# yzhang511/multi_modal_foundation_model

Hardware: AMD Instinct MI355X
Metric: pretrain samples/sec (T=100 bins/modality, d_model=256, 5+5 layers, spike+behaviour masked pretraining step) (higher is better)
Workload: dtype bf16; 1 GPU; BASELINE.json configs[1]: 1 session, ap(668 neurons)+behaviour(2), d_model=256, heads=8, mlp=512, 5 enc + 5 dec layers, T=100 (L=200 tokens), dropout 0.4/0.2, AdamW+OneCycleLR, mixed objectives; per_gpu_batch=1024, global_batch=1024, seq_len=200, parallelism=dp1

## Files before the change

### include/mmfm.h

```cpp
#ifndef MMFM_H
#define MMFM_H
#include <stdint.h>
#ifdef __cplusplus
extern "C" {
#endif

#define MMFM_VERSION 401
#define MMFM_F32 0
#define MMFM_BF16 1
#define MMFM_NULL_BIAS 1
#define MMFM_EMBED_OPTS 1
#define MMFM_MLP_GELU 0
#define MMFM_MLP_RELU 1
#define MMFM_MLP_SIGMOID 2
#define MMFM_MLP_GELU_TANH 3

typedef void* mmfm_stream;

typedef struct {
    const void* state;
    uint32_t site;
    float p;
} mmfm_dropout;

// ... 179 lines not shown
    int K, N;
    const void* x; int ldx;
    const void* w; int ldw;
    const float* bias;
    int ln; float eps;
    void* xhat; float* rstd;
    const void* residual; int ldr;
    void* y; int ldy;
    int stream_out;
    int rotate;
    int ln_bwd;
    const void* bwd_xhat; const float* bwd_rstd;
} mmfm_rowgemm_desc;
int mmfm_rowgemm(const mmfm_rowgemm_desc* d, mmfm_stream stream);

typedef struct {
    int64_t R;
    const void* x; int ldx;
    float eps;
    const void* w_up; const float* b_up;
    const void* w_down; const float* b_down;
    mmfm_dropout drop;
    void* y; int ldy;
    void* xhat; float* rstd;
    const void* dy; int lddy;
    const void* w_down_t;
    const void* w_up_t;
    void* t1; void* g; void* du;
    void* dx; int lddx;
    int rotate;
// ... 22 lines not shown
```

### multi_modal_foundation_model_amd/_lib.py

```python
from __future__ import annotations

import ctypes as C
import os
import re

import torch

_HERE = os.path.dirname(os.path.abspath(__file__))
LIB_PATH = os.environ.get("MMFM_LIB") or os.path.join(_HERE, "libmmfm_hip.so")
HEADER_PATH = os.path.join(os.path.dirname(_HERE), "include", "mmfm.h")

F32, BF16 = 0, 1
ATTN_DIAG, ATTN_CAUSAL, ATTN_SEP = 1, 2, 4
ACT_NONE, ACT_GELU, ACT_SOFTSIGN, ACT_GELU_GRAD, ACT_SOFTSIGN_GRAD, ACT_SOFTSIGN_GRAD_OUT = 0, 1, 2, 3, 4, 5
ACT_RELU, ACT_RELU_GRAD, ACT_SIGMOID, ACT_SIGMOID_GRAD, ACT_GELU_TANH, ACT_GELU_TANH_GRAD = 6, 7, 8, 9, 10, 11
(ACT_EMB_IDENTITY, ACT_EMB_IDENTITY_GRAD, ACT_EMB_RELU, ACT_EMB_RELU_GRAD, ACT_EMB_GELU, ACT_EMB_GELU_GRAD, ACT_EMB_SILU, ACT_EMB_SILU_GRAD,
 ACT_EMB_QUICK_GELU, ACT_EMB_QUICK_GELU_GRAD, ACT_EMB_GELU_TANH, ACT_EMB_GELU_TANH_GRAD, ACT_EMB_TANH, ACT_EMB_TANH_GRAD) = range(12, 26)
MLP_GELU, MLP_RELU, MLP_SIGMOID, MLP_GELU_TANH = 0, 1, 2, 3
LOSS_POISSON_LOG, LOSS_MSE, LOSS_POISSON_RATE, LOSS_L1, LOSS_SMOOTH_L1, LOSS_HUBER, LOSS_BCE_LOGITS = range(7)
LOSS_FULL = 1


class MmfmError(RuntimeError):
    pass
# ... 38 lines not shown
                ("WpP", C.c_void_p), ("WpTP", C.c_void_p)]


class ReduceEntry(C.Structure):
    _fields_ = [("dst", C.c_void_p), ("src", C.c_void_p), ("n", C.c_int64), ("slab_stride", C.c_int64), ("nslabs", C.c_int32),
                ("accumulate", C.c_int32), ("chunk0", C.c_int32), ("pad_", C.c_int32)]


class RowGemmDesc(C.Structure):
    _fields_ = [("R", C.c_int64), ("K", C.c_int), ("N", C.c_int), ("x", C.c_void_p), ("ldx", C.c_int), ("w", C.c_void_p),
                ("ldw", C.c_int), ("bias", C.c_void_p), ("ln", C.c_int), ("eps", C.c_float), ("xhat", C.c_void_p),
                ("rstd", C.c_void_p), ("residual", C.c_void_p), ("ldr", C.c_int), ("y", C.c_void_p), ("ldy", C.c_int),
                ("stream_out", C.c_int), ("rotate", C.c_int), ("ln_bwd", C.c_int), ("bwd_xhat", C.c_void_p), ("bwd_rstd", C.c_void_p)]


class MlpDesc(C.Structure):
    _fields_ = [("R", C.c_int64), ("x", C.c_void_p), ("ldx", C.c_int), ("eps", C.c_float), ("w_up", C.c_void_p),
                ("b_up", C.c_void_p), ("w_down", C.c_void_p), ("b_down", C.c_void_p), ("drop", Dropout), ("y", C.c_void_p),
                ("ldy", C.c_int), ("xhat", C.c_void_p), ("rstd", C.c_void_p), ("dy", C.c_void_p), ("lddy", C.c_int),
                ("w_down_t", C.c_void_p), ("w_up_t", C.c_void_p), ("t1", C.c_void_p), ("g", C.c_void_p), ("du", C.c_void_p),
                ("dx", C.c_void_p), ("lddx", C.c_int), ("rotate", C.c_int), ("scalenorm", C.c_int),
                ("act", C.c_int), ("act_beta", C.c_float)]


_vp, _i, _i64, _f = C.c_void_p, C.c_int, C.c_int64, C.c_float
_PROTOS = {
    "mmfm_version": (C.c_int, []),
    "mmfm_last_error": (C.c_char_p, []),
    "mmfm_device_check": (C.c_int, [_i]),
    "mmfm_rng_seed": (C.c_int, [_vp, C.c_uint64, _vp]),
# ... 24 lines not shown
    "mmfm_stitch_fwd_live": (C.c_int, [_i, _vp, _vp, _vp, _vp, _vp, _vp, _vp, _vp, _i, _i, _i, _i, _i, _i, _vp]),
    "mmfm_stitch_bwd_live": (C.c_int, [_i, _vp, _vp, _vp, _vp, _vp, Dropout, _vp, _vp, _vp, _i, _i, _i, _i, _i, _i, _i, _i, _vp, _i64, _vp]),
    "mmfm_stitch_bwd_workspace": (C.c_int64, [_i, _i, _i, _i, _i, _i]),
    "mmfm_stitch_bwd": (C.c_int, [_i, _vp, _vp, _vp, _vp, Dropout, _vp, _vp, _vp, _i, _i, _i, _i, _i, _i, _i, _i, _vp, _i64, _vp]),
    "mmfm_masked_loss_workspace": (C.c_int64, [_i64, _i]),
    "mmfm_masked_loss_fwd": (C.c_int, [_i, _i, _vp, _vp, _vp, _i, _i, _i64, _i, _vp, _vp, _i64, _vp]),
    "mmfm_masked_loss_kind_fwd": (C.c_int, [_i, _i, _f, _i, _vp, _vp, _vp, _i, _i, _i64, _i, _vp, _vp, _i64, _vp]),
    "mmfm_loss_finalize": (C.c_int, [_vp, _vp, _i, _vp, _vp, _vp]),
    "mmfm_masked_loss_bwd": (C.c_int, [_i, _i, _vp, _vp, _vp, _i, _i, _i64, _i, _vp, _vp, _vp, _vp]),
    "mmfm_masked_loss_kind_bwd": (C.c_int, [_i, _i, _f, _i, _vp, _vp, _vp, _i, _i, _i64, _i, _vp, _vp, _vp, _vp]),
    "mmfm_dropout_apply": (C.c_int, [_i, _vp, _vp, _i64, _i, Dropout, _vp]),
    "mmfm_cast_f32_to_bf16": (C.c_int, [_vp, _vp, _i64, _vp]),
    "mmfm_adamw_step": (C.c_int, [_vp, _vp, _vp, _vp, _vp, _i64, _vp, _vp]),
    "mmfm_prep_weights": (C.c_int, [_vp, _i, _i, _vp]),
    "mmfm_rowgemm": (C.c_int, [C.POINTER(RowGemmDesc), _vp]),
    "mmfm_mlp_fwd": (C.c_int, [C.POINTER(MlpDesc), _vp]),
    "mmfm_mlp_bwd": (C.c_int, [C.POINTER(MlpDesc), _vp]),
    "mmfm_ln_linear_grad_workspace": (C.c_int64, [_i]),
    "mmfm_ln_linear_grad": (C.c_int, [_vp, _vp, _vp, _vp, _i, _i, _vp, _vp, _vp, _vp, _i, _vp, _i64, _vp]),
    "mmfm_sn_linear_grad": (C.c_int, [_vp, _vp, _vp, _i, _i, _vp, _vp, _vp, _i, _vp, _i64, _vp]),
    "mmfm_r2_series": (C.c_int, [_vp, C.POINTER(_i64), _vp, C.POINTER(_i64), _i, _i, _i, _vp, _vp]),
    "mmfm_bits_per_spike_workspace": (C.c_int64, [_i64, _i]),
    "mmfm_bits_per_spike": (C.c_int, [_vp, _vp, _i64, _i, _vp, _vp, _i64, _vp]),
    "mmfm_bits_per_spike_neurons_workspace": (C.c_int64, [_i64, _i]),
    "mmfm_bits_per_spike_neurons": (C.c_int, [_vp, _vp, _i64, _i, _vp, _vp, _i64, _vp]),
    "mmfm_mt19937_jump": (C.c_int, [_vp, C.POINTER(C.c_int32), C.c_uint64]),
    "mmfm_mt19937_jump_reset": (C.c_int, []),
}

_lib = None
# ... 27 lines not shown
```

### multi_modal_foundation_model_amd/csrc/rowgemm.hip

```cpp
#define MMFM_ACT_LOAD_AUX 2
#include "rowchain.h"
#include <stdlib.h>
#include <algorithm>
#include <type_traits>

using namespace rowchain;

namespace {

constexpr int NT = 256, NW = 4;

constexpr int BIAS_MAX = 1024;

template <int KP, int LN, bool NTS, int NWV>
__global__ __launch_bounds__(NWV * 64, (KP == 1 ? 2 : 1)) void rowgemm_kernel(const mmfm_rowgemm_desc d) {
    constexpr int NT = NWV * 64, NW = NWV;
    __shared__ __attribute__((aligned(16))) char smem[LDS_BYTES + NW * STG_BYTES + BIAS_MAX * 4];
    const int t = threadIdx.x, lane = t & 63, wave = __builtin_amdgcn_readfirstlane(t >> 6), m = lane & 31, h = lane >> 5;
    const int npair = d.N >> 6, cpp = 2 * npair * KP;
    const int64_t npass = (d.R + 32 * NW - 1) / (32 * NW);
    const int my_passes = blockIdx.x < npass ? (int)((npass - 1 - blockIdx.x) / gridDim.x) + 1 : 0;
    if (my_passes == 0) return;
    const uint16_t* W = reinterpret_cast<const uint16_t*>(d.w);
    const int ldw = d.ldw;
// ... 407 lines not shown
            stage_lines(stg, rl, lane);
            f32x16 o[2];
#pragma unroll
            for (int j = 0; j < 2; ++j) {
                const f32x16 r = unstage_tile(stg, j, m, h);
#pragma unroll
                for (int i = 0; i < 16; ++i) o[j][i] = r[i] + rs * (acc[2 * q + j][i] - s1 - xt[2 * q + j][i] * s2);
            }
            stage_tile(stg, 0, m, h, o[0]);
            stage_tile(stg, 1, m, h, o[1]);
            flush_lines<false>(stg, Y, wrow0, ldyb, 128u * (2 * half + q), lane);
        }
    }
}

__global__ __launch_bounds__(256) void prep_weights_kernel(const mmfm_prep_entry* __restrict__ E, int ne) {
    __shared__ float tile[32][33];
    int e = 0;
    while (e + 1 < ne && (int)blockIdx.x >= E[e + 1].tile0) ++e;
    const mmfm_prep_entry en = E[e];
    const int n0 = ((int)blockIdx.x - en.tile0) * 32;
    const int tx = threadIdx.x & 31, ty = threadIdx.x >> 5;
    uint16_t* Wp = reinterpret_cast<uint16_t*>(en.Wp);
    uint16_t* WpT = reinterpret_cast<uint16_t*>(en.WpT);
    uint16_t* WpP = reinterpret_cast<uint16_t*>(en.WpP);
    uint16_t* WpTP = reinterpret_cast<uint16_t*>(en.WpTP);
    auto perm = [](int i) { return (i & ~12) | ((i & 4) << 1) | ((i & 8) >> 1); };
    float dot[4] = {0.f, 0.f, 0.f, 0.f};
    const float gs = en.scalar_gain ? en.gamma[0] : 1.f;
    for (int k0 = 0; k0 < en.K; k0 += 32) {
// ... 110 lines not shown
                    grid.y = (unsigned)((np_all + (np_all + ny - 1) / ny - 1) / ((np_all + ny - 1) / ny));
                    if (d.ln == 2) RGA_LAUNCH2(2, 0)
                    else if (d.ln) RGA_LAUNCH2(1, 0)
                    else RGA_LAUNCH2(0, 0)
                }
#undef RGA_LAUNCH2
#undef RGA_LAUNCH
            } else if (d.ln == 2) { RG_LAUNCH(1, 2) } else if (d.ln) { RG_LAUNCH(1, 1) } else { RG_LAUNCH(1, 0) }
        }
#undef RG_LAUNCH
    }
    MMFM_LAUNCH_CHECK("mmfm_rowgemm");
    return 0;
}

extern "C" int mmfm_prep_weights(const mmfm_prep_entry* entries_dev, int n_entries, int total_tiles, mmfm_stream stream) {
    MMFM_REQUIRE(entries_dev && n_entries > 0 && total_tiles > 0, "mmfm_prep_weights: empty table");
    hipLaunchKernelGGL(prep_weights_kernel, dim3(total_tiles), dim3(256), 0, (hipStream_t)stream, entries_dev, n_entries);
    MMFM_LAUNCH_CHECK("mmfm_prep_weights");
    return 0;
}
```

### multi_modal_foundation_model_amd/ops.py

```python
from __future__ import annotations

import ctypes as C

import torch

from . import _lib as L


def _stream():
    return torch.cuda.current_stream().cuda_stream


def run_plan(plan, stream=None):
    st = _stream() if stream is None else stream
    for fn, args, _keep in plan:
        rc = fn(*args, st)
        if rc:
            L.check(rc, fn.__name__)


def _emit(plan, fn, args, keep=()):
    if plan is None:
        L.check(fn(*args, _stream()), fn.__name__)
    else:
# ... 239 lines not shown
def prep_weights(table, n, tiles, plan=None):
    _emit(plan, L.lib().mmfm_prep_weights, (P(table), n, tiles), keep=(table,))


def rowgemm(x, w, y, R, N, K, *, ldx=None, ldw=None, ldy=None, bias=None, ln=False, eps=1e-5, xhat=None, rstd=None, residual=None,
            ldr=0, stream_out=False, ln_bwd=False, bwd_xhat=None, bwd_rstd=None, rotate=True, plan=None):
    d = L.RowGemmDesc()
    d.R, d.K, d.N = R, K, N
    d.x, d.ldx, d.w, d.ldw = P(x), K if ldx is None else ldx, P(w), K if ldw is None else ldw
    d.bias, d.ln, d.eps, d.xhat, d.rstd = P(bias), int(ln), eps, P(xhat), P(rstd)
    d.residual, d.ldr, d.y, d.ldy = P(residual), ldr, P(y), N if ldy is None else ldy
    d.stream_out, d.ln_bwd, d.bwd_xhat, d.bwd_rstd, d.rotate = int(stream_out), int(ln_bwd), P(bwd_xhat), P(bwd_rstd), int(rotate)
    _emit(plan, L.lib().mmfm_rowgemm, (C.byref(d),), keep=(d,))


MLP_ACTS = {
    "gelu": (L.MLP_GELU, 1.0),
    "relu": (L.MLP_RELU, 1.0),
    "silu": (L.MLP_SIGMOID, 1.0), "swish": (L.MLP_SIGMOID, 1.0), "quick_gelu": (L.MLP_SIGMOID, 1.702),
    "gelu_new": (L.MLP_GELU_TANH, 1.0), "gelu_pytorch_tanh": (L.MLP_GELU_TANH, 1.0), "gelu_fast": (L.MLP_GELU_TANH, 1.0),
}
GEMM_ACTS = {L.MLP_GELU: (L.ACT_GELU, L.ACT_GELU_GRAD), L.MLP_RELU: (L.ACT_RELU, L.ACT_RELU_GRAD),
             L.MLP_SIGMOID: (L.ACT_SIGMOID, L.ACT_SIGMOID_GRAD), L.MLP_GELU_TANH: (L.ACT_GELU_TANH, L.ACT_GELU_TANH_GRAD)}


EMBED_ACTS = {
    "softsign": (L.ACT_SOFTSIGN, L.ACT_SOFTSIGN_GRAD),
    "identity": (L.ACT_EMB_IDENTITY, L.ACT_EMB_IDENTITY_GRAD), "linear": (L.ACT_EMB_IDENTITY, L.ACT_EMB_IDENTITY_GRAD),
    "relu": (L.ACT_EMB_RELU, L.ACT_EMB_RELU_GRAD),
    "gelu": (L.ACT_EMB_GELU, L.ACT_EMB_GELU_GRAD),
# ... 67 lines not shown
```

### multi_modal_foundation_model_amd/plan.py

```python
from __future__ import annotations

import functools
import math
import os
from collections import namedtuple

import torch

from . import _lib as L
from . import ops as K


def _align(n, a=8):
    return (n + a - 1) // a * a


Switches = namedtuple("Switches", "fused gemm_big gemm_dw batch_reduce dw_pair attn_keepbits mlp_bwd_split")


def read_switches() -> Switches:
    env, on = os.environ, lambda k: os.environ.get(k, "1") != "0"
    return Switches(fused=int(env["MMFM_FUSED"]) if "MMFM_FUSED" in env else None, gemm_big=on("MMFM_GEMM_BIG"), gemm_dw=on("MMFM_GEMM_DW"),
                    batch_reduce=on("MMFM_BATCH_REDUCE"), dw_pair=on("MMFM_DW_PAIR"), attn_keepbits=on("MMFM_ATTN_KEEPBITS"),
                    mlp_bwd_split=env.get("MMFM_MLP_BWD_SPLIT", "1") == "1")


LIVE_ROWS_MIN = 16384


def live_rows_on(BT):
    v = os.environ.get("MMFM_LIVE_ROWS")
    return v == "1" if v in ("0", "1") else BT >= max(8192, LIVE_ROWS_MIN)


class Side:
    def __init__(self, sc, training):
        self.heads, self.I, self.act, self.scale, self.mult, self.max_F = sc.heads, sc.inter, sc.act, sc.embed_scale, sc.mult, sc.max_F
        self.dp, self.dpe = (sc.dropout, sc.embed_dropout) if training else (0.0, 0.0)
        self.act_fwd, self.act_grad = K.GEMM_ACTS[sc.act[0]]
        self.emb_act, self.pos = sc.embed_act, sc.embed_pos
        self.emb_fwd, self.emb_grad = K.embed_act(sc.embed_act)
        self.use_keep = self.F_MLP = False


class PlanBuilder:
    def __init__(self, engine, B, T, training, grad=True):
        e, c = self.e, self.c = engine, engine.cfg
# ... 90 lines not shown
        if self.batch_red:
            seg_max = max(end - s0 for _, s0, end in e.layout.segments)
            self.slabm = buf("ws/slabm", (max(1, min(R // 256, 15)) * (seg_max + 128 * 64),), f32)
        maxN = max([3 * H, self.Imax] + [n * self.mult_max for n in chans])
        buf("ws/col", (max(1, L.lib().mmfm_colsum_workspace(R, maxN) // 4),), f32)
        buf("ws/ln", (max(1, L.lib().mmfm_layernorm_bwd_workspace(R, H) // 4),), f32)
        buf("ws/stitch", (max(1, max(L.lib().mmfm_stitch_bwd_workspace(self.code, B, T, Lq, H, sd.max_F) for sd in self.sides.values()) // 4),), f32)
        buf("ws/loss", (max(1, L.lib().mmfm_masked_loss_workspace(BT, 1) // 4),), f32)
        self.pair_ok = self.code == L.BF16 and not self.batch_red and sw.dw_pair and sw.gemm_dw
        fm = self.fm = e._fused_mask(R, sw)
        self.F_QKV, self.F_LNL, self.F_OUT = bool(fm & 1), bool(fm & 2), bool(fm & 8)
        for name, sd in self.sides.items():
            sd.use_keep = self.code == L.BF16 and sd.dp > 0 and self.grad and sw.attn_keepbits
            sd.F_MLP = e.fused_mlp(name, fm)
        self.prep = e._build_prep() if fm else None
        if fm:
            K.prep_weights(self.prep["table"], self.prep["n"], self.prep["tiles"], plan=self.fwd)
            self.gdb = buf("ws/gdb", (max(_align(l.N * l.K + l.N) for l in e.linears if l.norm),), f32)
            if "ws/lng" not in self.b:
                self.b["ws/lng"] = K.ln_linear_grad_workspace(H, e.device)

    def slab_region(self, S, stride):
        o = self.slabm_off
        self.slabm_off = o + S * stride
        if self.slabm_off > self.slabm.numel():
            raise RuntimeError(f"engine: ws/slabm holds {self.slabm.numel()} floats, the plan's slab regions need {self.slabm_off}")
        return self.slabm[o:o + S * stride]

    def lin(self, plan, X, wname, Y, Mr, N, Kd, ldx=None, live=None, **kw):
        gemm = K.gemm if live is None else functools.partial(K.gemm_live, live=live)
# ... 223 lines not shown
                    K.stitch_fwd_live(tok_tmp, mod_row, pos, b["ts"], b[mk(side, "keep0")], lv._keep, xs, es_, B, T, Lq, slot, H, sd.max_F, plan=fwd)
                else:
                    K.stitch_fwd(tok_tmp, mod_row, pos, b["ts"], b[mk(side, "keep0")], xs, es_, B, T, Lq, slot, H, sd.max_F, plan=fwd)
        X = x_enc
        for i in range(c.n_enc):
            p, tag = f"encoder.{i}", f"enc{i}"
            self.stream_in[tag] = X
            X = self.mlp_block(fwd, self.self_block(fwd, X, p, tag, self.enc_flags), p, tag)
        self.enc_last = X
        enc_out, context = buf("enc_out", (R, H)), buf("context", (R, H))
        if self.F_LNL:
            self.ln_lin(fwd, X, "encoder_norm", "decoder_proj_context", context, H, "encnorm", residual=emb_enc)
        else:
            self.ln_f(fwd, X, "encoder_norm", enc_out, "encnorm")
            self.lin(fwd, enc_out, "decoder_proj_context", context, R, H, H, residual=emb_enc, ldr=H)
        Y = x_dec
        for i in range(c.n_dec):
            p, tag = f"decoder.{i}", f"dec{i}"
            self.stream_in[tag] = Y
            Ya = self.self_block(fwd, Y, p, tag, self.dec_flags)
            qc, kvc, a2, Yb = buf(tag + "/qc", (R, H)), buf(tag + "/kvc", (R, 2 * H)), buf(tag + "/a2", (R, H)), buf(tag + "/yb", (R, H))
            if self.F_LNL:
                self.ln_lin(fwd, Ya, p + ".query_norm", p + ".cross_attn.query", qc, H, tag + "/qn")
                self.ln_lin(fwd, context, p + ".context_norm", p + ".cross_attn.kv", kvc, 2 * H, tag + "/cn", alias=None if i == 0 else "dec0/cn")
            else:
                hq, hc = buf(tag + "/hq", (R, H)), buf(tag + "/hc", (R, H))
                self.ln_f(fwd, Ya, p + ".query_norm", hq, tag + "/qn")
                self.ln_f(fwd, context, p + ".context_norm", hc, tag + "/cn")
                self.lin(fwd, hq, p + ".cross_attn.query", qc, R, H, H)
                self.lin(fwd, hc, p + ".cross_attn.kv", kvc, R, 2 * H, H)
            K.attn_fwd(self.attn_desc(tag + "/xa", qc, H, kvc, 2 * H, 0, H, a2, self.enc_flags), plan=fwd)
            self.out_proj(fwd, a2, p + ".cross_attn.out_proj", Ya, Yb)
            Y = self.mlp_block(fwd, Yb, p, tag)
        self.dec_last = Y
        ydec = buf("ydec", (R, H))
        self.ln_f(fwd, Y, "decoder_norm", ydec, "decnorm", ds_L=Lq, ds_T=T)
        tokmask = b[mk("decoder", "tokmask")]
        for j, (m, mod, n) in enumerate(self.mods_of["decoder"]):
            pred = buf(f"pred/{m}", (BT, n))
            self.lin(fwd, ydec[j * BT:(j + 1) * BT], f"decoder_embeddings.{mod}.out", pred, BT, n, H)
            self.loss(fwd, mod, K.masked_loss_fwd, K.masked_loss_kind_fwd, pred, b[f"tgt/{m}"], tokmask[:, j * T:], Lq, T, BT, n,
                      b["loss_sum"][j:j + 1], b["ws/loss"])
        K.loss_finalize(b["loss_sum"], b[mk("decoder", "count")], M, b["loss"], b["inv_n"], plan=fwd)

    def close_segment(self, name):
        if self.pend:
            K.reduce_slabs_multi(list(self.pend), self.e.device, plan=self.cur)
            self.pend.clear()
        for g_site, wname, lnname, N in self.late_lng:
            self.lin_norm_grad(self.cur, g_site, wname, lnname, N)
        self.late_lng.clear()
        self.slabm_off = 0
        self.bwd.append((name, self.cur))
        self.cur = []

    def mlp_back(self, plan, dS, p, tag, X_in):
        e, b, buf, R, H, sd = self.e, self.b, self.buf, self.R, self.H, self.side(p)
        I, dp = sd.I, sd.dp
# ... 34 lines not shown
        if self.F_OUT:
            self.dlin(plan, dS, a, wname, R, H, H, defer=True)
            K.rowgemm(dS, self.prep["v"][wname]["WpT"], t2, R, H, H, plan=plan)
        else:
            self.dlin(plan, dS, a, wname, R, H, H, dX=t2)

    def self_back(self, plan, dS, p, tag, flags):
        b, H = self.b, self.H
        self.out_proj_back(plan, dS, b[tag + "/a"], p + ".attn.out_proj")
        qkv, dqkv = b[tag + "/qkv"], b["d/qkv"]
        K.attn_bwd(self.attn_desc(tag + "/sa", qkv, 3 * H, qkv, 3 * H, H, 2 * H, b[tag + "/a"], flags, d_o=b["d/t2"], dq=dqkv, dkv=dqkv,
                                  lddq=3 * H, lddkv=3 * H, dkoff=H, dvoff=2 * H), plan=plan)
        self.norm_lin_back(plan, self.F_QKV, dqkv, 3 * H, tag + "/ln1", p + ".attn.qkv", p + ".ln1", tag + "/h1", self.stream_in[tag], dS, dS)

    def cross_back(self, plan, dY, p, tag, dctx_in):
        b, H, dqc, dkvc = self.b, self.H, self.b["d/qc"], self.b["d/kvc"]
        self.out_proj_back(plan, dY, b[tag + "/a2"], p + ".cross_attn.out_proj")
        K.attn_bwd(self.attn_desc(tag + "/xa", b[tag + "/qc"], H, b[tag + "/kvc"], 2 * H, 0, H, b[tag + "/a2"], self.enc_flags,
                                  d_o=b["d/t2"], dq=dqc, dkv=dkvc, lddq=H, lddkv=2 * H, dkoff=0, dvoff=H), plan=plan)
        self.norm_lin_back(plan, self.F_LNL, dqc, H, tag + "/qn", p + ".cross_attn.query", p + ".query_norm", tag + "/hq", b[tag + "/xa"], dY, dY)
        self.norm_lin_back(plan, self.F_LNL, dkvc, 2 * H, tag + "/cn", p + ".cross_attn.kv", p + ".context_norm", tag + "/hc", b["context"],
                           dctx_in, b["d/ctx"])

    def backward(self):
        e, c, b, buf = self.e, self.c, self.b, self.buf
        B, T, H, I, R, BT, Lq = self.B, self.T, self.H, self.Imax, self.R, self.BT, self.Lq
        dY, dydec = buf("d/stream", (R, H)), buf("d/ydec", (R, H))
        buf("d/t1", (R, H)); buf("d/t2", (R, H)); buf("d/h", (R, H)); buf("d/u", (R, I)); buf("d/qkv", (R, 3 * H)); dctx = buf("d/ctx", (R, H))
        ydec = b["ydec"]
        tokmask = b[self.mk("decoder", "tokmask")]
        for j, (m, mod, n) in enumerate(self.mods_of["decoder"]):
            dpred = buf(f"d/pred/{m}", (BT, n))
            self.loss(self.cur, mod, K.masked_loss_bwd, K.masked_loss_kind_bwd, b[f"pred/{m}"], b[f"tgt/{m}"], tokmask[:, j * T:],
                      Lq, T, BT, n, b["gout"], b["inv_n"], dpred)
            self.dlin(self.cur, dpred, ydec[j * BT:(j + 1) * BT], f"decoder_embeddings.{mod}.out", BT, n, H, dX=dydec[j * BT:(j + 1) * BT])
        self.ln_b(self.cur, dydec, self.dec_last, "decoder_norm", "decnorm", None, dY, ds_L=Lq, ds_T=T)
        self.close_segment("head")
        buf("d/qc", (R, H)); buf("d/kvc", (R, 2 * H))
        for i in reversed(range(c.n_dec)):
            p, tag = f"decoder.{i}", f"dec{i}"
            self.mlp_back(self.cur, dY, p, tag, b[tag + "/yb"])
            self.cross_back(self.cur, dY, p, tag, None if i == c.n_dec - 1 else dctx)
            self.self_back(self.cur, dY, p, tag, self.dec_flags)
            self.close_segment(p)
        if c.n_dec == 0:
            raise NotImplementedError("n_dec == 0")
        dX = buf("d/xstream", (R, H))
        self.norm_lin_back(self.cur, self.F_LNL, dctx, H, "encnorm", "decoder_proj_context", "encoder_norm", "enc_out", self.enc_last, None, dX)
        self.close_segment("bridge")
        for i in reversed(range(c.n_enc)):
            p, tag = f"encoder.{i}", f"enc{i}"
            self.mlp_back(self.cur, dX, p, tag, b[tag + "/xa"])
            self.self_back(self.cur, dX, p, tag, self.enc_flags)
            self.close_segment(p)
        shared = {mod for _, mod, _ in self.mods_of["decoder"] if c.mod_emb_owner("decoder", mod) == "encoder"}
        for side, dS, dextra in (("decoder", dY, None), ("encoder", dX, dctx)):
            sd = self.sides[side]
            for slot, (m, mod, n) in enumerate(self.mods_of[side]):
                pS = f"{side}_embeddings.{mod}.embedder"
                lv = self.lv.get((side, slot))
                stitch = K.stitch_bwd if lv is None else functools.partial(K.stitch_bwd_live, rec=lv._keep)
                stitch(dS, dextra, b["ts"], b[self.mk(side, "keep0")], drop=e._drop(f"{side}/embdrop/{m}", sd.dpe), d_tok=buf(f"d/tok/{side}/{m}", (BT, H)),
# ... 23 lines not shown
```

Before: 36130 samples/s.

## Group decoder cross-attention context KV projections into one norm-fused grouped GEMM

Adds a grouped row-GEMM kernel that normalises the encoder context once and projects it through all decoder layers' cross-attention KV weights in one launch. A matching backward kernel sums every layer's dKV through the transposed weights and the context-norm backward into dctx in one pass. This is meant to remove repeated reads and normalisation of the context, and the per-layer accumulation into dctx. The cost is separate per-layer dKV buffers, which add memory. It also forces every decoder layer's context_norm to be the same norm kind. It is on by default when the row count is at least 16384.

```diff
diff --git a/include/mmfm.h b/include/mmfm.h
--- a/include/mmfm.h
+++ b/include/mmfm.h
@@ -217,6 +217,24 @@
 } mmfm_rowgemm_desc;
 int mmfm_rowgemm(const mmfm_rowgemm_desc* d, mmfm_stream stream);
 
+#define MMFM_ROWGEMM_MAX_GROUPS 8
+typedef struct {
+    int64_t R;
+    int K, N;
+    int groups;
+    const void* x[MMFM_ROWGEMM_MAX_GROUPS]; int ldx;
+    const void* w[MMFM_ROWGEMM_MAX_GROUPS]; int ldw;
+    const float* bias[MMFM_ROWGEMM_MAX_GROUPS];
+    void* y[MMFM_ROWGEMM_MAX_GROUPS]; int ldy;
+    int ln; float eps;
+    void* xhat; float* rstd;
+    const void* residual; int ldr;
+    int stream_out, rotate;
+    int ln_bwd;
+    const void* bwd_xhat; const float* bwd_rstd;
+} mmfm_rowgemm_groups_desc;
+int mmfm_rowgemm_groups(const mmfm_rowgemm_groups_desc* d, mmfm_stream stream);
+
 typedef struct {
     int64_t R;
     const void* x; int ldx;
diff --git a/multi_modal_foundation_model_amd/_lib.py b/multi_modal_foundation_model_amd/_lib.py
--- a/multi_modal_foundation_model_amd/_lib.py
+++ b/multi_modal_foundation_model_amd/_lib.py
@@ -76,6 +76,17 @@
                 ("stream_out", C.c_int), ("rotate", C.c_int), ("ln_bwd", C.c_int), ("bwd_xhat", C.c_void_p), ("bwd_rstd", C.c_void_p)]
 
 
+ROWGEMM_MAX_GROUPS = 8
+
+
+class RowGemmGroupsDesc(C.Structure):
+    _fields_ = [("R", C.c_int64), ("K", C.c_int), ("N", C.c_int), ("groups", C.c_int), ("x", C.c_void_p * ROWGEMM_MAX_GROUPS), ("ldx", C.c_int),
+                ("w", C.c_void_p * ROWGEMM_MAX_GROUPS), ("ldw", C.c_int), ("bias", C.c_void_p * ROWGEMM_MAX_GROUPS),
+                ("y", C.c_void_p * ROWGEMM_MAX_GROUPS), ("ldy", C.c_int), ("ln", C.c_int), ("eps", C.c_float), ("xhat", C.c_void_p),
+                ("rstd", C.c_void_p), ("residual", C.c_void_p), ("ldr", C.c_int), ("stream_out", C.c_int), ("rotate", C.c_int),
+                ("ln_bwd", C.c_int), ("bwd_xhat", C.c_void_p), ("bwd_rstd", C.c_void_p)]
+
+
 class MlpDesc(C.Structure):
     _fields_ = [("R", C.c_int64), ("x", C.c_void_p), ("ldx", C.c_int), ("eps", C.c_float), ("w_up", C.c_void_p),
                 ("b_up", C.c_void_p), ("w_down", C.c_void_p), ("b_down", C.c_void_p), ("drop", Dropout), ("y", C.c_void_p),
@@ -130,6 +141,7 @@
     "mmfm_adamw_step": (C.c_int, [_vp, _vp, _vp, _vp, _vp, _i64, _vp, _vp]),
     "mmfm_prep_weights": (C.c_int, [_vp, _i, _i, _vp]),
     "mmfm_rowgemm": (C.c_int, [C.POINTER(RowGemmDesc), _vp]),
+    "mmfm_rowgemm_groups": (C.c_int, [C.POINTER(RowGemmGroupsDesc), _vp]),
     "mmfm_mlp_fwd": (C.c_int, [C.POINTER(MlpDesc), _vp]),
     "mmfm_mlp_bwd": (C.c_int, [C.POINTER(MlpDesc), _vp]),
     "mmfm_ln_linear_grad_workspace": (C.c_int64, [_i]),
diff --git a/multi_modal_foundation_model_amd/csrc/rowgemm.hip b/multi_modal_foundation_model_amd/csrc/rowgemm.hip
--- a/multi_modal_foundation_model_amd/csrc/rowgemm.hip
+++ b/multi_modal_foundation_model_amd/csrc/rowgemm.hip
@@ -445,6 +445,204 @@
     }
 }
 
+constexpr int GROUPS_MAX = MMFM_ROWGEMM_MAX_GROUPS;
+constexpr int GBIAS_MAX = 2560;
+struct GroupOff { uint32_t w[GROUPS_MAX]; };
+template <typename T>
+__device__ __forceinline__ T pick8(const T (&a)[GROUPS_MAX], int g) {
+    T r = a[0];
+#pragma unroll
+    for (int i = 1; i < GROUPS_MAX; ++i) r = g == i ? a[i] : r;
+    return r;
+}
+
+#pragma clang diagnostic push
+#pragma clang diagnostic ignored "-Winline-asm"
+template <int LN, bool NTS>
+__global__ __launch_bounds__(256, 2) void rowgemm_groups_a_kernel(const mmfm_rowgemm_groups_desc d, const void* wbase, const GroupOff wo, int nps) {
+    constexpr int NT = 256, NW = 4, RING_B = RINGA_SLOTS * CHUNK;
+    extern __shared__ __attribute__((aligned(16))) char smem[];
+    const int t = threadIdx.x, lane = t & 63, wave = __builtin_amdgcn_readfirstlane(t >> 6), m = lane & 31, h = lane >> 5;
+    const int np_g = d.N >> 6, np_all = np_g * d.groups;
+    const int npb = (np_all + (int)gridDim.y - 1) / (int)gridDim.y, pbase = (int)blockIdx.y * npb;
+    const int npair = min(npb, np_all - pbase), cpp = 2 * npair;
+    const int64_t npass = (d.R + 32 * NW - 1) / (32 * NW);
+    const int my_passes = blockIdx.x < npass ? (int)((npass - 1 - blockIdx.x) / gridDim.x) + 1 : 0;
+    if (my_passes == 0 || npair <= 0) return;
+    const __amdgpu_buffer_rsrc_t rs_w = wbuf(wbase);
+    const uint32_t ldwb = (uint32_t)d.ldw * 2u;
+    const int rot = d.rotate ? (int)(blockIdx.x % npair) : 0;
+    auto src = [&](int g) {
+        const int ti = g % cpp;
+        int vp = (ti >> 1) + rot; vp = pbase + (vp >= npair ? vp - npair : vp);
+        const int pr = vp & (np_g - 1);
+        AChunk c;
+        c.rs = rs_w; c.off = __builtin_amdgcn_readfirstlane(pick8(wo.w, vp >> nps) + (uint32_t)(32 * (2 * pr + (ti & 1))) * ldwb); c.ldb = ldwb; c.kind = 0;
+        return c;
+    };
+    char* stg = smem + RING_B + wave * STG_BYTES;
+    float* lbias = reinterpret_cast<float*>(smem + RING_B + NW * STG_BYTES);
+    for (int g = 0; g < d.groups; ++g) stage_vec(lbias + g * d.N, pick8(d.bias, g), d.N, t, NT);
+    const GBuf X = gbuf(d.x[0], d.R * d.ldx * 2);
+    const GBuf XH = gbuf(blockIdx.y == 0 ? d.xhat : nullptr, d.R * 512), RS = gbuf(blockIdx.y == 0 ? d.rstd : nullptr, d.R * 4);
+    const uint32_t ldxb = d.ldx * 2, ldyb = d.ldy * 2;
+    const ALane<NT> ring_al = alane_init<NT>(t, ldwb, 0u);
+    const AFrag fr = afrag_init(m, h);
+    RINGA_DECL(NT);
+    RINGA_START((uint32_t)(uintptr_t)(__attribute__((address_space(3))) char*)smem, my_passes * cpp, src);
+    for (int pi = 0; pi < my_passes; ++pi) {
+        const uint32_t wrow0 = (uint32_t)(((int64_t)(blockIdx.x + (int64_t)pi * gridDim.x) * NW + wave) * 32);
+        const bool live = wrow0 < (uint32_t)d.R;
+        opnd x[16];
+        if (live) {
+            load_rows_lines<4>(stg, x, X, wrow0, ldxb, lane, m, h);
+            const float rs = norm_rows<LN>(x, d.eps);
+            store_rows_lines<4, true>(stg, XH, wrow0, 512u, lane, m, h, x);
+            st4f(RS, h == 0 ? (wrow0 + m) * 4u : 0xfffffff0u, rs);
+        }
+        auto pair = [&](int tp, auto first) {
+            constexpr int EX = decltype(first)::value ? 0 : 4;
+            int vp = tp + rot; vp = pbase + (vp >= npair ? vp - npair : vp);
+            const int grp = vp >> nps, pr = vp & (np_g - 1);
+            const GBuf Y = gbuf(pick8(d.y, grp), d.R * d.ldy * 2);
+            const float* gb = lbias + grp * d.N;
+            f32x16 acc[2];
+#pragma unroll
+            for (int j = 0; j < 2; ++j) {
+                uint32_t slot;
+                if (live) vm_wait_n<1024 / NT + EX>(); else vm_wait_n<1024 / NT>();
+                RINGA_SYNC_NOWAIT(src, slot);
+                if (live) {
+                    acc[j] = mma16a<4>(slot, fr, x, zero16(), [&](int g_) { RINGA_PIECE(g_); });
+                    add_vec(acc[j], gb, 2 * pr + j, h);
+                } else {
+#pragma unroll
+                    for (int q = 0; q < 1024 / NT; ++q) RINGA_PIECE(q);
+                }
+            }
+            if (!live) return;
+            stage_tile(stg, 0, m, h, acc[0]);
+            stage_tile(stg, 1, m, h, acc[1]);
+            flush_lines<NTS>(stg, Y, wrow0, ldyb, 128u * pr, lane);
+        };
+        pair(0, std::true_type());
+        for (int tp = 1; tp < npair; ++tp) pair(tp, std::false_type());
+    }
+}
+
+template <int KP, int NORM>
+__global__ __launch_bounds__(NT) void rowgemm_groups_lnbwd_kernel(const mmfm_rowgemm_groups_desc d, const void* wbase, const GroupOff wo) {
+    constexpr int RING_B = RINGA_SLOTS * CHUNK;
+    extern __shared__ __attribute__((aligned(16))) char smem[];
+    const int t = threadIdx.x, lane = t & 63, wave = __builtin_amdgcn_readfirstlane(t >> 6), m = lane & 31, h = lane >> 5;
+    const int npiece = d.groups * KP;
+    const int64_t npass = (d.R + 32 * NW - 1) / (32 * NW);
+    const int my_passes = blockIdx.x < npass ? (int)((npass - 1 - blockIdx.x) / gridDim.x) + 1 : 0;
+    if (my_passes == 0) return;
+    const __amdgpu_buffer_rsrc_t rs_w = wbuf(wbase);
+    const uint32_t ldwb = (uint32_t)d.ldw * 2u;
+    int src_q = 0, src_t = 0;
+    auto src = [&](int) {
+        const int g = KP == 1 ? src_q : src_q >> 1, p = KP == 1 ? 0 : src_q & 1;
+        AChunk c;
+        c.rs = rs_w; c.off = __builtin_amdgcn_readfirstlane(pick8(wo.w, g) + (uint32_t)(32 * src_t) * ldwb + 512u * (uint32_t)p); c.ldb = ldwb; c.kind = 0;
+        if (++src_t == 8) { src_t = 0; if (++src_q == npiece) src_q = 0; }
+        return c;
+    };
+    char* stg = smem + RING_B + wave * STG_BYTES;
+    char* xstash = smem + RING_B + NW * STG_BYTES + wave * 4 * STG_BYTES;
+    const GBuf Y = gbuf(d.y[0], d.R * d.ldy * 2), RES = gbuf(d.residual, d.R * d.ldr * 2);
+    const GBuf XH = gbuf(d.bwd_xhat, d.R * 512), RS = gbuf(d.bwd_rstd, d.R * 4);
+    const uint32_t ldxb = d.ldx * 2, ldyb = d.ldy * 2, ldrb = d.ldr * 2;
+    const int64_t xbytes = d.R * d.ldx * 2;
+    const ALane<NT> ring_al = alane_init<NT>(t, ldwb, 0u);
+    const AFrag fr = afrag_init(m, h);
+    RINGA_DECL(NT);
+    RINGA_START((uint32_t)(uintptr_t)(__attribute__((address_space(3))) char*)smem, my_passes * 8 * npiece, src);
+    auto row_of = [&](int pi) { return (uint32_t)(((int64_t)(blockIdx.x + (int64_t)pi * gridDim.x) * NW + wave) * 32); };
+    opnd x[16];
+    load_rows_lines<4>(stg, x, gbuf(d.x[0], xbytes), row_of(0), ldxb, lane, m, h);
+    for (int pi = 0; pi < my_passes; ++pi) {
+        const uint32_t wrow0 = row_of(pi);
+        const uint32_t nrow0 = pi + 1 < my_passes ? row_of(pi + 1) : (uint32_t)(npass * 32 * NW);
+        {
+            Lines xl[4];
+#pragma unroll
+            for (int tp = 0; tp < 4; ++tp) xl[tp] = fetch_lines(XH, wrow0, 512u, 128u * tp, lane);
+#pragma unroll
+            for (int tp = 0; tp < 4; ++tp) stage_lines(xstash + tp * STG_BYTES, xl[tp], lane);
+        }
+        float rs = ld4f(RS, (wrow0 + m) * 4u);
+        f32x16 acc[8];
+#pragma unroll
+        for (int tt = 0; tt < 8; ++tt) acc[tt] = zero16();
+        for (int q = 0; q < npiece; ++q) {
+            const int nq = q + 1 < npiece ? q + 1 : 0;
+            const uint32_t nrow = q + 1 < npiece ? wrow0 : nrow0;
+            const GBuf XN = gbuf(pick8(d.x, KP == 1 ? nq : nq >> 1), xbytes);
+            const uint32_t ncol = KP == 1 ? 0u : 512u * (uint32_t)(nq & 1);
+            Lines L[4];
+#pragma unroll
+            for (int s = 0; s < 4; ++s) L[s] = fetch_lines(XN, nrow, ldxb, ncol + 128u * s, lane);
+            opnd xn[16];
+#pragma unroll
+            for (int tt = 0; tt < 8; ++tt) {
+                if (tt == 2) {
+#pragma unroll
+                    for (int s = 0; s < 4; ++s) {
+                        stage_lines(stg, L[s], lane);
+#pragma unroll
+                        for (int s4 = 0; s4 < 4; ++s4) xn[4 * s + s4] = unstage_opnd(stg, s4, m, h);
+                    }
+                }
+                uint32_t slot;
+                if (tt < 2) { RINGA_SYNC(src, slot, 16); acc[tt] = mma16a<4>(slot, fr, x, acc[tt], [&](int g_) { RINGA_PIECE(g_); }); }
+                else { RINGA_SYNC(src, slot, 0); acc[tt] = mma16a<4>(slot, fr, x, acc[tt], [&](int g_) { RINGA_PIECE(g_); }); }
+            }
+#pragma unroll
+            for (int s = 0; s < 16; ++s) x[s] = xn[s];
+        }
+        float s1 = 0.f, s2 = 0.f;
+#pragma unroll
+        for (int tp = 0; tp < 4; ++tp) {
+#pragma unroll
+            for (int j = 0; j < 2; ++j) {
+                const f32x16 xt = unstage_tile(xstash + tp * STG_BYTES, j, m, h);
+#pragma unroll
+                for (int i = 0; i < 16; ++i) { s1 += acc[2 * tp + j][i]; s2 = fmaf(acc[2 * tp + j][i], xt[i], s2); }
+            }
+        }
+        s1 = xhalf(s1);
+        s2 = xhalf(s2);
+        norm_bwd_stats<NORM>(s1, s2, rs);
+        Lines rl4[4];
+#pragma unroll
+        for (int tp = 0; tp < 4; ++tp) rl4[tp] = fetch_lines(RES, wrow0, ldrb, 128u * tp, lane);
+#pragma unroll
+        for (int tp = 0; tp < 4; ++tp) {
+            const Lines& rl = rl4[tp];
+            f32x16 o[2];
+#pragma unroll
+            for (int j = 0; j < 2; ++j) {
+                const f32x16 xt = unstage_tile(xstash + tp * STG_BYTES, j, m, h);
+#pragma unroll
+                for (int i = 0; i < 16; ++i) o[j][i] = rs * (acc[2 * tp + j][i] - s1 - xt[i] * s2);
+            }
+            stage_lines(stg, rl, lane);
+#pragma unroll
+            for (int j = 0; j < 2; ++j) {
+                const f32x16 r = unstage_tile(stg, j, m, h);
+#pragma unroll
+                for (int i = 0; i < 16; ++i) o[j][i] += r[i];
+            }
+            stage_tile(stg, 0, m, h, o[0]);
+            stage_tile(stg, 1, m, h, o[1]);
+            flush_lines<false>(stg, Y, wrow0, ldyb, 128u * tp, lane);
+        }
+    }
+}
+#pragma clang diagnostic pop
+
 __global__ __launch_bounds__(256) void prep_weights_kernel(const mmfm_prep_entry* __restrict__ E, int ne) {
     __shared__ float tile[32][33];
     int e = 0;
@@ -585,6 +783,76 @@
     return 0;
 }
 
+extern "C" int mmfm_rowgemm_groups(const mmfm_rowgemm_groups_desc* dp, mmfm_stream stream) {
+    const mmfm_rowgemm_groups_desc d = *dp;
+    MMFM_REQUIRE(d.groups >= 1 && d.groups <= GROUPS_MAX && d.R > 0, "mmfm_rowgemm_groups: groups = %d (1 .. %d), R = %lld", d.groups, GROUPS_MAX, (long long)d.R);
+    MMFM_REQUIRE(d.ln >= 0 && d.ln <= 2 && d.ln_bwd >= 0 && d.ln_bwd <= 2 && (d.ln != 0) != (d.ln_bwd != 0),
+                 "mmfm_rowgemm_groups: ln = %d, ln_bwd = %d: exactly one of them must be 1 (LayerNorm) or 2 (ScaleNorm)", d.ln, d.ln_bwd);
+    MMFM_REQUIRE(d.ldx % 8 == 0 && d.ldw % 8 == 0 && d.ldy % 8 == 0 && d.ldx >= d.K && d.ldw >= d.K && d.ldy >= d.N,
+                 "mmfm_rowgemm_groups: leading dimensions (%d, %d, %d) must be multiples of 8 and cover the rows", d.ldx, d.ldw, d.ldy);
+    auto al16 = [](const void* p) { return ((uintptr_t)p & 15) == 0; };
+    const int nx = d.ln_bwd ? d.groups : 1, ny = d.ln_bwd ? 1 : d.groups;
+    uintptr_t wmin = (uintptr_t)d.w[0];
+    for (int g = 0; g < d.groups; ++g) {
+        MMFM_REQUIRE(d.w[g] && al16(d.w[g]) && al16(d.bias[g]), "mmfm_rowgemm_groups: group %d: weights NULL or operands not 16-byte aligned", g);
+        MMFM_REQUIRE(g >= nx || (d.x[g] && al16(d.x[g])), "mmfm_rowgemm_groups: group %d: x NULL or not 16-byte aligned", g);
+        MMFM_REQUIRE(g >= ny || (d.y[g] && al16(d.y[g])), "mmfm_rowgemm_groups: group %d: y NULL or not 16-byte aligned", g);
+        wmin = std::min(wmin, (uintptr_t)d.w[g]);
+    }
+    MMFM_REQUIRE(al16(d.residual) && al16(d.xhat) && al16(d.bwd_xhat), "mmfm_rowgemm_groups: operands must be 16-byte aligned");
+    GroupOff wo = {};
+    const int64_t wbytes = (int64_t)(d.ln_bwd ? 256 : d.N) * d.ldw * 2;
+    for (int g = 0; g < d.groups; ++g) {
+        const int64_t off = (int64_t)((uintptr_t)d.w[g] - wmin);
+        MMFM_REQUIRE(off + wbytes < (int64_t)1 << 31, "mmfm_rowgemm_groups: group %d: weights more than 2 GiB from the first group's", g);
+        wo.w[g] = (uint32_t)off;
+    }
+    const int64_t maxld = std::max<int64_t>(std::max(d.ldx, d.ldy), std::max(d.ldr, 256));
+    MMFM_REQUIRE((d.R + 256) * maxld * 2 < (int64_t)1 << 31, "mmfm_rowgemm_groups: tensors beyond 2 GiB are not addressable by the 32-bit buffer offsets");
+    static const int per_cu_env = [] { const char* e = getenv("MMFM_ROWGEMM_WG_PER_CU"); return e ? atoi(e) : 0; }();
+    hipStream_t st = (hipStream_t)stream;
+    const void* wbase = (const void*)wmin;
+    if (d.ln_bwd) {
+        MMFM_REQUIRE(d.N == 256 && (d.K == 256 || d.K == 512) && d.bwd_xhat && d.bwd_rstd,
+                     "mmfm_rowgemm_groups: ln_bwd needs N = 256, K = 256 or 512 (got %d, %d), x_hat and rstd", d.N, d.K);
+        MMFM_REQUIRE(!d.residual || (d.ldr % 8 == 0 && d.ldr >= d.N), "mmfm_rowgemm_groups: ldr %d", d.ldr);
+        dim3 grid(grid_for(d.R, per_cu_env > 0 ? per_cu_env : 1)), block(NT);
+        constexpr int LDS_L = RINGA_SLOTS * CHUNK + NW * STG_BYTES + NW * 4 * STG_BYTES;
+#define GLNB(KP, NORM)                                                                                                      \
+        {                                                                                                                   \
+            if (int rc = mmfm_lds_opt_in(reinterpret_cast<const void*>(rowgemm_groups_lnbwd_kernel<KP, NORM>), LDS_L, "mmfm_rowgemm_groups")) return rc; \
+            hipLaunchKernelGGL((rowgemm_groups_lnbwd_kernel<KP, NORM>), grid, block, LDS_L, st, d, wbase, wo);              \
+        }
+        if (d.K == 256) { if (d.ln_bwd == 2) GLNB(1, 2) else GLNB(1, 1) }
+        else { if (d.ln_bwd == 2) GLNB(2, 2) else GLNB(2, 1) }
+#undef GLNB
+    } else {
+        MMFM_REQUIRE(d.K == 256, "mmfm_rowgemm_groups: the norm prologue needs K = 256 (got %d)", d.K);
+        MMFM_REQUIRE(d.N >= 64 && d.N <= 1024 && (d.N & (d.N - 1)) == 0, "mmfm_rowgemm_groups: N = %d must be 64, 128, 256, 512 or 1024", d.N);
+        MMFM_REQUIRE(d.groups * d.N <= GBIAS_MAX, "mmfm_rowgemm_groups: groups * N = %d > %d", d.groups * d.N, GBIAS_MAX);
+        MMFM_REQUIRE(!d.residual, "mmfm_rowgemm_groups: the grouped forward takes no residual");
+        int nps = 0;
+        while ((64 << nps) < d.N) ++nps;
+        dim3 grid(grid_for(d.R, per_cu_env > 0 ? per_cu_env : 2, 4)), block(256);
+        constexpr int LDS_A = RINGA_SLOTS * CHUNK + 4 * STG_BYTES + GBIAS_MAX * 4;
+        const int64_t npass = (d.R + 127) / 128;
+        const int np_all = (d.N >> 6) * d.groups;
+        static const int nsplit_env = [] { const char* e = getenv("MMFM_ROWGEMM_NSPLIT"); return e ? atoi(e) : 1; }();
+        const int nyb = (nsplit_env && npass < 128) ? (int)std::max<int64_t>(1, std::min<int64_t>(np_all, 512 / npass)) : 1;
+        grid.y = (unsigned)((np_all + (np_all + nyb - 1) / nyb - 1) / ((np_all + nyb - 1) / nyb));
+#define GFWD(LN, NTS)                                                                                                       \
+        {                                                                                                                   \
+            if (int rc = mmfm_lds_opt_in(reinterpret_cast<const void*>(rowgemm_groups_a_kernel<LN, NTS>), LDS_A, "mmfm_rowgemm_groups")) return rc; \
+            hipLaunchKernelGGL((rowgemm_groups_a_kernel<LN, NTS>), grid, block, LDS_A, st, d, wbase, wo, nps);              \
+        }
+        if (d.ln == 2) { if (d.stream_out) GFWD(2, true) else GFWD(2, false) }
+        else { if (d.stream_out) GFWD(1, true) else GFWD(1, false) }
+#undef GFWD
+    }
+    MMFM_LAUNCH_CHECK("mmfm_rowgemm_groups");
+    return 0;
+}
+
 extern "C" int mmfm_prep_weights(const mmfm_prep_entry* entries_dev, int n_entries, int total_tiles, mmfm_stream stream) {
     MMFM_REQUIRE(entries_dev && n_entries > 0 && total_tiles > 0, "mmfm_prep_weights: empty table");
     hipLaunchKernelGGL(prep_weights_kernel, dim3(total_tiles), dim3(256), 0, (hipStream_t)stream, entries_dev, n_entries);
diff --git a/multi_modal_foundation_model_amd/ops.py b/multi_modal_foundation_model_amd/ops.py
--- a/multi_modal_foundation_model_amd/ops.py
+++ b/multi_modal_foundation_model_amd/ops.py
@@ -277,6 +277,29 @@
     _emit(plan, L.lib().mmfm_rowgemm, (C.byref(d),), keep=(d,))
 
 
+def rowgemm_groups(xs, ws, ys, R, N, K, *, ldx=None, ldw=None, ldy=None, biases=None, ln=False, eps=1e-5, xhat=None, rstd=None,
+                   residual=None, ldr=0, stream_out=False, ln_bwd=False, bwd_xhat=None, bwd_rstd=None, rotate=True, plan=None):
+    G = len(ws)
+    if not 1 <= G <= L.ROWGEMM_MAX_GROUPS:
+        raise ValueError(f"rowgemm_groups: {G} groups (1 .. {L.ROWGEMM_MAX_GROUPS})")
+    if len(xs) != (G if ln_bwd else 1) or len(ys) != (1 if ln_bwd else G):
+        raise ValueError("rowgemm_groups: forward takes one x and a y per group, backward an x per group and one y")
+    d = L.RowGemmGroupsDesc()
+    d.R, d.K, d.N, d.groups = R, K, N, G
+    for g in range(G):
+        d.w[g] = P(ws[g])
+        d.bias[g] = P(biases[g]) if biases is not None else None
+    for g, x in enumerate(xs):
+        d.x[g] = P(x)
+    for g, y in enumerate(ys):
+        d.y[g] = P(y)
+    d.ldx, d.ldw, d.ldy = K if ldx is None else ldx, K if ldw is None else ldw, N if ldy is None else ldy
+    d.ln, d.eps, d.xhat, d.rstd = int(ln), eps, P(xhat), P(rstd)
+    d.residual, d.ldr = P(residual), ldr
+    d.stream_out, d.ln_bwd, d.bwd_xhat, d.bwd_rstd, d.rotate = int(stream_out), int(ln_bwd), P(bwd_xhat), P(bwd_rstd), int(rotate)
+    _emit(plan, L.lib().mmfm_rowgemm_groups, (C.byref(d),), keep=(d,))
+
+
 MLP_ACTS = {
     "gelu": (L.MLP_GELU, 1.0),
     "relu": (L.MLP_RELU, 1.0),
diff --git a/multi_modal_foundation_model_amd/plan.py b/multi_modal_foundation_model_amd/plan.py
--- a/multi_modal_foundation_model_amd/plan.py
+++ b/multi_modal_foundation_model_amd/plan.py
@@ -31,6 +31,15 @@
 def live_rows_on(BT):
     v = os.environ.get("MMFM_LIVE_ROWS")
     return v == "1" if v in ("0", "1") else BT >= max(8192, LIVE_ROWS_MIN)
+
+
+CTX_GROUP_MIN = 16384
+CTX_GROUP_BIAS = 2560
+
+
+def ctx_group_on(R):
+    v = os.environ.get("MMFM_CTX_GROUP")
+    return v == "1" if v in ("0", "1") else R >= CTX_GROUP_MIN
 
 
 class Side:
@@ -151,6 +160,7 @@
             sd.use_keep = self.code == L.BF16 and sd.dp > 0 and self.grad and sw.attn_keepbits
             sd.F_MLP = e.fused_mlp(name, fm)
         self.prep = e._build_prep() if fm else None
+        self.ctx_group = self.F_LNL and self.code == L.BF16 and c.n_dec > 0 and ctx_group_on(R)
         if fm:
             K.prep_weights(self.prep["table"], self.prep["n"], self.prep["tiles"], plan=self.fwd)
             self.gdb = buf("ws/gdb", (max(_align(l.N * l.K + l.N) for l in e.linears if l.norm),), f32)
@@ -404,6 +414,8 @@
         else:
             self.ln_f(fwd, X, "encoder_norm", enc_out, "encnorm")
             self.lin(fwd, enc_out, "decoder_proj_context", context, R, H, H, residual=emb_enc, ldr=H)
+        if self.ctx_group:
+            self.context_kv(fwd, context)
         Y = x_dec
         for i in range(c.n_dec):
             p, tag = f"decoder.{i}", f"dec{i}"
@@ -412,7 +424,8 @@
             qc, kvc, a2, Yb = buf(tag + "/qc", (R, H)), buf(tag + "/kvc", (R, 2 * H)), buf(tag + "/a2", (R, H)), buf(tag + "/yb", (R, H))
             if self.F_LNL:
                 self.ln_lin(fwd, Ya, p + ".query_norm", p + ".cross_attn.query", qc, H, tag + "/qn")
-                self.ln_lin(fwd, context, p + ".context_norm", p + ".cross_attn.kv", kvc, 2 * H, tag + "/cn", alias=None if i == 0 else "dec0/cn")
+                if not self.ctx_group:
+                    self.ln_lin(fwd, context, p + ".context_norm", p + ".cross_attn.kv", kvc, 2 * H, tag + "/cn", alias=None if i == 0 else "dec0/cn")
             else:
                 hq, hc = buf(tag + "/hq", (R, H)), buf(tag + "/hc", (R, H))
                 self.ln_f(fwd, Ya, p + ".query_norm", hq, tag + "/qn")
@@ -432,6 +445,36 @@
             self.loss(fwd, mod, K.masked_loss_fwd, K.masked_loss_kind_fwd, pred, b[f"tgt/{m}"], tokmask[:, j * T:], Lq, T, BT, n,
                       b["loss_sum"][j:j + 1], b["ws/loss"])
         K.loss_finalize(b["loss_sum"], b[mk("decoder", "count")], M, b["loss"], b["inv_n"], plan=fwd)
+
+    def ctx_norm_kind(self):
+        kinds = {self.e.is_sn(f"decoder.{i}.context_norm") for i in range(self.c.n_dec)}
+        assert len(kinds) == 1, "decoder layers with different context_norm kinds"
+        return 2 if kinds.pop() else 1
+
+    def context_kv(self, plan, context):
+        b, R, H, n_dec = self.b, self.R, self.H, self.c.n_dec
+        per = max(1, min(L.ROWGEMM_MAX_GROUPS, CTX_GROUP_BIAS // (2 * H)))
+        xh = rs = None
+        if self.grad:
+            xh, rs = self.buf("dec0/cn/xh", (R, H)), self.buf("dec0/cn/rs", (R,), torch.float32)
+        for i0 in range(0, n_dec, per):
+            ids = range(i0, min(n_dec, i0 + per))
+            pws = [self.prep["v"][f"decoder.{i}.cross_attn.kv"] for i in ids]
+            K.rowgemm_groups([context], [pw["Wp"] for pw in pws], [self.buf(f"dec{i}/kvc", (R, 2 * H)) for i in ids], R, 2 * H, H,
+                             biases=[pw["bp"] for pw in pws], ln=self.ctx_norm_kind(), xhat=xh if i0 == 0 else None,
+                             rstd=rs if i0 == 0 else None, stream_out=True, plan=plan)
+        if self.grad:
+            for i in range(1, n_dec):
+                b[f"dec{i}/cn/xh"], b[f"dec{i}/cn/rs"] = xh, rs
+
+    def context_back(self, plan, dctx):
+        b, R, H, n_dec = self.b, self.R, self.H, self.c.n_dec
+        order = list(reversed(range(n_dec)))
+        for j0 in range(0, n_dec, L.ROWGEMM_MAX_GROUPS):
+            ids = order[j0:j0 + L.ROWGEMM_MAX_GROUPS]
+            K.rowgemm_groups([b[f"d/kvc/{i}"] for i in ids], [self.prep["v"][f"decoder.{i}.cross_attn.kv"]["WpT"] for i in ids], [dctx], R, H, 2 * H,
+                             ldw=2 * H, residual=dctx if j0 else None, ldr=H if j0 else 0, ln_bwd=self.ctx_norm_kind(),
+                             bwd_xhat=b["dec0/cn/xh"], bwd_rstd=b["dec0/cn/rs"], plan=plan)
 
     def close_segment(self, name):
         if self.pend:
@@ -496,11 +539,16 @@
         self.norm_lin_back(plan, self.F_QKV, dqkv, 3 * H, tag + "/ln1", p + ".attn.qkv", p + ".ln1", tag + "/h1", self.stream_in[tag], dS, dS)
 
     def cross_back(self, plan, dY, p, tag, dctx_in):
-        b, H, dqc, dkvc = self.b, self.H, self.b["d/qc"], self.b["d/kvc"]
+        b, H, dqc = self.b, self.H, self.b["d/qc"]
+        dkvc = b["d/kvc/" + tag[3:]] if self.ctx_group else b["d/kvc"]
         self.out_proj_back(plan, dY, b[tag + "/a2"], p + ".cross_attn.out_proj")
         K.attn_bwd(self.attn_desc(tag + "/xa", b[tag + "/qc"], H, b[tag + "/kvc"], 2 * H, 0, H, b[tag + "/a2"], self.enc_flags,
                                   d_o=b["d/t2"], dq=dqc, dkv=dkvc, lddq=H, lddkv=2 * H, dkoff=0, dvoff=H), plan=plan)
         self.norm_lin_back(plan, self.F_LNL, dqc, H, tag + "/qn", p + ".cross_attn.query", p + ".query_norm", tag + "/hq", b[tag + "/xa"], dY, dY)
+        if self.ctx_group:
+            self.dlin_ln(plan, dkvc, tag + "/cn", p + ".cross_attn.kv", p + ".context_norm", 2 * H)
+            self.flush_deferred(plan)
+            return
         self.norm_lin_back(plan, self.F_LNL, dkvc, 2 * H, tag + "/cn", p + ".cross_attn.kv", p + ".context_norm", tag + "/hc", b["context"],
                            dctx_in, b["d/ctx"])
 
@@ -518,7 +566,12 @@
             self.dlin(self.cur, dpred, ydec[j * BT:(j + 1) * BT], f"decoder_embeddings.{mod}.out", BT, n, H, dX=dydec[j * BT:(j + 1) * BT])
         self.ln_b(self.cur, dydec, self.dec_last, "decoder_norm", "decnorm", None, dY, ds_L=Lq, ds_T=T)
         self.close_segment("head")
-        buf("d/qc", (R, H)); buf("d/kvc", (R, 2 * H))
+        buf("d/qc", (R, H))
+        if self.ctx_group:
+            for i in range(c.n_dec):
+                buf(f"d/kvc/{i}", (R, 2 * H))
+        else:
+            buf("d/kvc", (R, 2 * H))
         for i in reversed(range(c.n_dec)):
             p, tag = f"decoder.{i}", f"dec{i}"
             self.mlp_back(self.cur, dY, p, tag, b[tag + "/yb"])
@@ -528,6 +581,8 @@
         if c.n_dec == 0:
             raise NotImplementedError("n_dec == 0")
         dX = buf("d/xstream", (R, H))
+        if self.ctx_group:
+            self.context_back(self.cur, dctx)
         self.norm_lin_back(self.cur, self.F_LNL, dctx, H, "encnorm", "decoder_proj_context", "encoder_norm", "enc_out", self.enc_last, None, dX)
         self.close_segment("bridge")
         for i in reversed(range(c.n_enc)):
```

Result: faster. 36620 samples/s, median of 6 (+1.4%).
